# inhavl-shlee/AFI-GAN

Hardware: AMD Instinct MI355X
Metric: stage1_G+D_step_images_per_s (higher is better)
Workload: dtype f32 via f16x3: two scaled fp16 pieces per operand, three f16 MFMAs per product, fp32 accumulate (tensors fp32)

## Files before the change

### afigan_amd/csrc/nets.hip

```cpp
#include <string.h>
#include <stdlib.h>

#include "../../include/afigan_hip.h"
#include "afi_common.h"
#include "afi_launch.h"
#include <initializer_list>
#include <new>


#include <vector>
namespace {
struct SideStream {
    hipStream_t side = nullptr;
    std::vector<hipEvent_t> ring;
    size_t next = 0;
    bool init() {
        if (side) return true;
        if (hipStreamCreateWithFlags(&side, hipStreamNonBlocking) != hipSuccess) { side = nullptr; return false; }
        ring.resize(128);
        for (auto& e : ring)
            if (hipEventCreateWithFlags(&e, hipEventDisableTiming) != hipSuccess) return false;
        return true;
    }
    void destroy() {
// ... 247 lines not shown
    int nj = 0;
    long long used = 0;
    for (int i = 0; i < n; ++i) {
        const Wk6Req& r = reqs[i];
        const long long need = wk6_req_floats(r.Ncols, r.Ck, r.nKphase);
        bool hit = false;
        float* slot = wino_wcache_slot(cx, r.key,  4 + r.tag, r.nKphase, r.Ncols, r.Ck, need, hit);
        if (!slot) {
            if (!arena || used + need > arena_floats) { im.n = 0; return AFI_OK; }
            slot = arena + used; used += need; hit = false;
        }
        const int nst = afi_cdiv(r.Ck, 32) * 9 * r.nKphase;
        if (!hit && r.convT) {
            if (have_ct) { im.n = 0; return AFI_OK; }
            ct = AfiWk6ConvT{r.j[0].src, (unsigned char*)slot, r.pack_dst, r.convT == 1 ? r.Ck : r.Ncols, r.convT == 1 ? r.Ncols / 4 : r.Ck, r.convT == 1 ? 0 : 1, 0};
            have_ct = true;
        } else if (!hit) {
            int chunk0 = 0;
            for (int k = 0; k < r.njob; ++k) {
                if (nj == kWk6MaxJobs) { im.n = 0; return AFI_OK; }
                jobs[nj++] = AfiWk6ImgJob{r.j[k].src, r.j[k].b_sRow, r.j[k].b_sTap, r.Ncols, r.j[k].Ck, 9, r.nKphase, r.b_rc, chunk0 * 9 * r.nKphase,
                                          (unsigned char*)slot, r.njob > 1 ? nst : 0, 0};
                chunk0 += afi_cdiv(r.j[k].Ck, 32);
            }
        }
        im.e[im.n++] = Wk6Images::Ent{r.key, r.tag, (const unsigned char*)slot, nst};
    }
    if (nj || have_ct) {
        AFI_TRY(afi_launch_wk6_images(jobs, nj, st, side, have_ct ? &ct : nullptr));
        if (side && side_done) *side_done = true;
        if (have_ct && ct_built) *ct_built = true;
    }
    rollback.keep = true;
    im.on = true;
    return AFI_OK;
}
static inline bool wk6_shapes_ok(int C, int G, int R) { return (C % 32) == 0 && (G % 32) == 0 && 6 * R + 4 <= kWk6MaxReq && 9 * R + 4 <= kWk6MaxJobs; }
constexpr long long kWk6HiResMaxPixels = 4096;
static long long gen_wk6_fwd_floats(int C, int G, int R, long long P) {
    if (P > kWk6MaxPixels || !wk6_shapes_ok(C, G, R)) return 0;
    const int L = C + 4 * G;
    long long f = 3 * wk6_req_floats(C, C, 1) + wk6_req_floats(4 * C, C, 1);
    for (int k = 1; k <= 4; ++k) f += (long long)R * wk6_req_floats(G, C + (k - 1) * G, 1);
    return f + (long long)R * wk6_req_floats(C, L, 1);
}
static long long gen_wk6_bwd_floats(int C, int G, int R, long long P) {
    if (P > kWk6MaxPixels || !wk6_shapes_ok(C, G, R)) return 0;
    const int L = C + 4 * G;
    long long f = 3 * wk6_req_floats(C, C, 1) + wk6_req_floats(C, C, 4);
    for (int k = 1; k <= 4; ++k) f += (long long)R * wk6_req_floats(C + (k - 1) * G, G, 1);
    return f + (long long)R * (wk6_req_floats(L, C, 1) + wk6_req_floats(C, 4 * G, 1));
}

static int wino_run(afi_ctx* cx, const AfiPixGemm& g, const WinoForm& f, float* ws, long long ws_floats, float* part, long long part_floats, hipStream_t st) {
    AFI_TRY(afi_o16_refused(g));
    const int b_rc = f.kind == kWinoDgrad;
    const int nph = g.nKphase;
    const int K = g.Ck * nph, Nc = g.Ncols;
    if (ws_floats < wino_ws_floats(g.N, g.H, g.W, K, Nc)) return AFI_ERR_WORKSPACE;
    const int dtype = f.dtype, np = f.np; const long long Tpad = f.Tpad;
    const bool f4 = f.f4, dma = f.dma, f16 = f.f16;
    float* U = ws;
    float* Vb = U + align4((long long)np * K * Nc);
    float* Mb = Vb + align4(np * Tpad * K);
    float* Usp = Mb + align4(np * Tpad * Nc);
    float* amax = nullptr;
    bool have_u = false;
    if (g.no_wcache) {
    } else if (dma) {
        if (float* slot = wino_wcache_slot(cx, g.B, f4, b_rc | (dtype << 4), b_rc ? K : Nc, b_rc ? Nc : K, wino_usplit_floats(np, (long long)K * Nc), have_u)) Usp = slot;
    } else if (float* slot = wino_wcache_slot(cx, g.B, f4, b_rc, b_rc ? K : Nc, b_rc ? Nc : K, align4((long long)np * K * Nc), have_u)) U = slot;
    if (!have_u) {
        float* wmax = dma && f16 ? afi_f16_image_wmax(Usp) : nullptr;
        if (wmax) AFI_TRY(afi_f16_image_begin(Usp, st));
        AFI_TRY(f4 ? afi_launch_wino4_weight(g.B, U, b_rc ? K : Nc, b_rc ? Nc : K, b_rc, st, wmax)
                   : afi_launch_wino_weight(g.B, U, b_rc ? K : Nc, b_rc ? Nc : K, b_rc, st, wmax));
        if (dma) AFI_TRY(f16 ? afi_launch_split_f16_tiles(U, Usp, np, Nc, K, st, f4 ? 6 : 5) : afi_launch_split_bf16_tiles(U, Usp, np, Nc, K, dtype, st));
    }
    const bool a_pre = f.presplit && g.a_amax && g.a_amax_known;
    if (f16 && !(amax = g.a_amax ? g.a_amax : wino_amax_take(cx, ws, ws_floats, 1, st))) return AFI_ERR_LAUNCH;
    const AfiF16Bound abound = afi_f16_bound(amax, f4 ? 2 : 1);
    if (g.v_keep && !(f.keep && a_pre)) return AFI_ERR_BAD_ARG;
    if (g.v_keep) Vb = g.v_keep;
    for (int ph = 0; ph < nph; ++ph) {
        AfiView a = g.A;
        if (nph == 4) { a.p += (ph >> 1) * g.A.sH + (ph & 1) * g.A.sW; a.sH *= 2; a.sW *= 2; }
        float* raise = g.a_amax ? (g.a_amax_known ? nullptr : g.a_amax) : (f16 ? amax : nullptr);
        AFI_TRY(f4 ? afi_launch_wino4_input(a, g.N, g.H, g.W, g.Ck, Tpad, Vb + ph * g.Ck, st, K, &g.a_bn, raise, a_pre ? &abound : nullptr)
                   : afi_launch_wino_input(a, g.N, g.H, g.W, g.Ck, Tpad, Vb + ph * g.Ck, st, K, &g.a_bn, raise, a_pre ? &abound : nullptr));
    }
    if (dma) {
        if (f16) AFI_TRY(afi_launch_gemm_nt_f16x3(Vb, Usp, Mb, np, Tpad, Nc, K, abound, st, a_pre, afi_opt(cx, AFI_OPT_F16_NT256_MIN_TILES), g.nt_local_sums != 0));
        else AFI_TRY(afi_launch_gemm_nt_bf16_dma(Vb, Usp, Mb, np, Tpad, Nc, K, dtype, st));
        return f4 ? afi_launch_wino4_output_epi(Mb, Tpad, g, st) : afi_launch_wino_output_epi(Mb, Tpad, g, st);
    }
    if (dtype == AFI_DTYPE_F32) {
        const int rc = afi_launch_gemm_nt(Vb, U, Mb, np, Tpad, Nc, K, st);
        if (rc == AFI_OK) return f4 ? afi_launch_wino4_output_epi(Mb, Tpad, g, st) : afi_launch_wino_output_epi(Mb, Tpad, g, st);
        if (rc != AFI_ERR_UNSUPPORTED) return rc;
    }
    AfiPixGemm q = pix_default(np, 1, (int)Tpad);
    q.ntaps = 1; q.Ck = K; q.Ncols = Nc; q.CoutPhase = Nc;
    q.A = AfiView{Vb, Tpad * K, 0, K};
    q.B = U; q.b_sRow = K; q.b_sTap = 0; q.b_sImg = (long long)K * Nc;
    q.n_fastest = 1;
    q.O = AfiView{Mb, Tpad * Nc, 0, Nc};
    q.partial = part; q.partial_floats = part_floats;
    AFI_TRY(afi_launch_pix_gemm(q, 0, st));
    return f4 ? afi_launch_wino4_output_epi(Mb, Tpad, g, st) : afi_launch_wino_output_epi(Mb, Tpad, g, st);
}

struct AfiBwdSums { double* rows; const float* c; AfiBnLoad bn; float slope; };
struct WinoConvOpt {
    double* stats = nullptr; float* stats_mm = nullptr; int* stats_rows = nullptr;
    const AfiBnLoad* in_bn = nullptr;
    float* in_amax = nullptr; bool in_amax_known = false;
    float* v_keep = nullptr;
    bool local_sums = false;
    const AfiBwdSums* bsums = nullptr; int* bsums_rows = nullptr;
};
static int wino_conv(afi_ctx* cx, WinoKind kind, AfiView in, int N, int H, int W, int K, const float* w, int Nc, const float* bias, AfiView out, AfiView z,
// ... 281 lines not shown
    AFI_CTX_CHECK(ctx);
    if (out_dtype != AFI_STORE_BF16 && out_dtype != AFI_STORE_F16) return AFI_ERR_BAD_ARG;
    if ((Cin & 3) || (Cout & 3)) return AFI_ERR_UNSUPPORTED;
    AfiPixGemm g = conv_fwd_desc(V(x), N, H, W, Cin, w, bias, Cout, V(out));
    g.alpha = alpha; g.beta = beta; g.lrelu = lrelu; g.o_dtype = out_dtype;
    return launch_pix_op(cx, g, 0, (hipStream_t)stream);
}
int afi_conv3x3_dgrad(afi_ctx_t* ctx, afi_view_t dy, int N, int H, int W, int Cout, const float* w, int Cin, afi_view_t dx, float alpha, float beta,
                      afi_view_t z, void* stream) {
    afi_ctx* cx = ctx; (void)cx;
    AFI_CTX_CHECK(ctx);
    if ((Cin & 3) || (Cout & 3)) return AFI_ERR_UNSUPPORTED;
    AfiPixGemm g = conv_dgrad_desc(V(dy), N, H, W, Cout, w, Cin, V(dx));
    g.alpha = alpha; g.beta = beta;
    if (z.p) { g.Z = V(z); g.z_lo = 0; g.z_hi = Cin; }
    return launch_pix_op(cx, g, 1, (hipStream_t)stream);
}
int afi_conv3x3_wgrad(afi_ctx_t* ctx, afi_view_t dy, afi_view_t x, int N, int H, int W, int Cout, int Cin, float* dw, float alpha, void* stream) {
    afi_ctx* cx = ctx; (void)cx;
    AFI_CTX_CHECK(ctx);
    if ((Cin & 3) || (Cout & 3)) return AFI_ERR_UNSUPPORTED;
    return wgrad_launch(cx, conv_wgrad_desc(V(dy), V(x), N, H, W, Cout, Cin, dw, alpha), (hipStream_t)stream);
}

long long afi_conv3x3_wino_ws_floats(int N, int H, int W, int Cin, int Cout) { return wino_ws_floats(N, H, W, Cin, Cout); }
int afi_conv3x3_wino_fwd(afi_ctx_t* ctx, afi_view_t x, int N, int H, int W, int Cin, const float* w, const float* bias, int Cout, afi_view_t out, float* ws,
                         long long ws_floats, void* stream) {
    afi_ctx* cx = ctx; (void)cx;
    AFI_CTX_CHECK(ctx);
    if (N <= 0 || H <= 0 || W <= 0 || !ws) return AFI_ERR_BAD_ARG;
    return wino_conv(cx, kWinoFwd, V(x), N, H, W, Cin, w, Cout, bias, V(out), null_view(), ws, ws_floats, nullptr, 0, (hipStream_t)stream);
}
int afi_conv3x3_wino_fwd_out16(afi_ctx_t* ctx, afi_view_t x, int N, int H, int W, int Cin, const float* w, const float* bias, int Cout, afi_view_t out,
                               int out_dtype, float* ws, long long ws_floats, void* stream) {
    afi_ctx* cx = ctx; (void)cx;
    AFI_CTX_CHECK(ctx);
    if (out_dtype != AFI_STORE_BF16 && out_dtype != AFI_STORE_F16) return AFI_ERR_BAD_ARG;
    if (N <= 0 || H <= 0 || W <= 0 || !ws) return AFI_ERR_BAD_ARG;
    if ((Cin & 3) || (Cout & 3)) return AFI_ERR_UNSUPPORTED;
    AfiPixGemm g = conv_fwd_desc(V(x), N, H, W, Cin, w, bias, Cout, V(out));
    g.o_dtype = out_dtype;
    return wino_run(cx, g, wino_form(cx, g, 0), ws, ws_floats, nullptr, 0, (hipStream_t)stream);
}
int afi_conv3x3_wino_infer(afi_ctx_t* ctx, afi_view_t x, int N, int H, int W, int Cin, const float* w, const float* bias, int Cout, afi_view_t out, int act,
                           float* ws, long long ws_floats, void* stream) {
    afi_ctx* cx = ctx; (void)cx;
    AFI_CTX_CHECK(ctx);
    if (N <= 0 || H <= 0 || W <= 0 || !ws || act < 0 || act > 2) return AFI_ERR_BAD_ARG;
    if ((Cin & 3) || (Cout & 3)) return AFI_ERR_UNSUPPORTED;
    AfiPixGemm g = conv_fwd_desc(V(x), N, H, W, Cin, w, bias, Cout, V(out));
    g.lrelu = act;
    return wino_run(cx, g, wino_form(cx, g, 0, true), ws, ws_floats, nullptr, 0, (hipStream_t)stream);
}
int afi_conv3x3_wino_dgrad(afi_ctx_t* ctx, afi_view_t dy, int N, int H, int W, int Cout, const float* w, int Cin, afi_view_t dx, afi_view_t z, float* ws,
                           long long ws_floats, void* stream) {
    afi_ctx* cx = ctx; (void)cx;
    AFI_CTX_CHECK(ctx);
    if (N <= 0 || H <= 0 || W <= 0 || !ws) return AFI_ERR_BAD_ARG;
    return wino_conv(cx, kWinoDgrad, V(dy), N, H, W, Cout, w, Cin, nullptr, V(dx), z.p ? V(z) : null_view(), ws, ws_floats, nullptr, 0, (hipStream_t)stream);
}

int afi_conv3x3_wino_wgrad(afi_ctx_t* ctx, afi_view_t dy, afi_view_t x, int N, int H, int W, int Cout, int Cin, float* dw, float alpha, float* ws,
                           long long ws_floats, void* stream) {
    afi_ctx* cx = ctx; (void)cx;
    AFI_CTX_CHECK(ctx);
    if (N <= 0 || H <= 0 || W <= 0 || !ws || !dw) return AFI_ERR_BAD_ARG;
    return wino_wgrad(cx, V(dy), V(x), N, H, W, Cout, Cin, dw, alpha, ws, ws_floats, (hipStream_t)stream);
}

int afi_conv1x1_fwd(afi_ctx_t* ctx, afi_view_t x, int N, int H, int W, int Cin, const float* w, const float* bias, int Cout, afi_view_t out, float alpha,
                    float beta, afi_view_t r1, float r1_scale, int lrelu, void* stream) {
    afi_ctx* cx = ctx; (void)cx;
    AFI_CTX_CHECK(ctx);
    if ((Cin & 3) || (Cout & 3)) return AFI_ERR_UNSUPPORTED;
    AfiPixGemm g = pix_default(N, H, W);
    g.ntaps = 1; g.Ck = Cin; g.Ncols = Cout; g.CoutPhase = Cout;
    g.A = V(x); g.B = w; g.b_sRow = Cin; g.b_sTap = 0;
    g.O = V(out); g.bias = bias; g.alpha = alpha; g.beta = beta; g.lrelu = lrelu;
    if (r1.p) { g.R1 = V(r1); g.r1s = r1_scale; g.r1_lo = 0; g.r1_hi = Cout; }
    return launch_pix_op(cx, g, 0, (hipStream_t)stream);
}
int afi_conv1x1_dgrad(afi_ctx_t* ctx, afi_view_t dy, int N, int H, int W, int Cout, const float* w, int Cin, afi_view_t dx, float alpha, float beta,
                      void* stream) {
    afi_ctx* cx = ctx; (void)cx;
    AFI_CTX_CHECK(ctx);
    if ((Cin & 3) || (Cout & 3)) return AFI_ERR_UNSUPPORTED;
    AfiPixGemm g = pix_default(N, H, W);
    g.ntaps = 1; g.a_sgn = -1; g.Ck = Cout; g.Ncols = Cin; g.CoutPhase = Cin;
    g.A = V(dy); g.B = w; g.b_sRow = Cin; g.b_sTap = 0;
    g.O = V(dx); g.alpha = alpha; g.beta = beta;
    return launch_pix_op(cx, g, 1, (hipStream_t)stream);
}
int afi_conv1x1_dgrad_out16(afi_ctx_t* ctx, afi_view_t dy, int N, int H, int W, int Cout, const float* w, int Cin, afi_view_t dx, int dx_dtype, float alpha,
                            float beta, void* stream) {
    afi_ctx* cx = ctx; (void)cx;
    AFI_CTX_CHECK(ctx);
    if (dx_dtype != AFI_STORE_BF16 && dx_dtype != AFI_STORE_F16) return AFI_ERR_BAD_ARG;
    if ((Cin & 3) || (Cout & 3)) return AFI_ERR_UNSUPPORTED;
    AfiPixGemm g = pix_default(N, H, W);
    g.ntaps = 1; g.a_sgn = -1; g.Ck = Cout; g.Ncols = Cin; g.CoutPhase = Cin;
    g.A = V(dy); g.B = w; g.b_sRow = Cin; g.b_sTap = 0;
    g.O = V(dx); g.alpha = alpha; g.beta = beta; g.o_dtype = dx_dtype;
    return launch_pix_op(cx, g, 1, (hipStream_t)stream);
}
int afi_conv1x1_wgrad(afi_ctx_t* ctx, afi_view_t dy, afi_view_t x, int N, int H, int W, int Cout, int Cin, float* dw, float alpha, void* stream) {
    afi_ctx* cx = ctx; (void)cx;
// ... 1133 lines not shown
```

### afigan_amd/guide.py

```python
import math

import torch
import torch.nn as nn
import torch.nn.functional as F

from . import ops


def _kaiming(shape, fan_in, gain=1.0):
    return torch.randn(shape) * (gain * math.sqrt(2.0 / fan_in))


class _Conv1x1(nn.Module):
    def __init__(self, cin, cout, stride=1, relu=False, gain=1.0):
        super().__init__()
        self.stride, self.relu = stride, relu
        self.register_buffer("w", _kaiming((cin, cout), cin, gain).t().contiguous())
        self.register_buffer("b", torch.zeros(cout))

    def forward(self, x, add=None, relu=None):
        if self.stride != 1:
            x = x[:, :, ::self.stride, ::self.stride]
        return ops.conv1x1_fwd(x, self.w, self.b, add=add, act=2 if (self.relu if relu is None else relu) else 0)


class _Conv3x3(nn.Module):
    def __init__(self, cin, cout, relu=False):
        super().__init__()
        self.relu = relu
        self.register_buffer("w", _kaiming((cout, 3, 3, cin), cin * 9).permute(0, 3, 1, 2))
        self.register_buffer("b", torch.zeros(cout))

    def forward(self, x):
        N, C, H, W = x.shape
        if C >= 128 and self.w.shape[0] >= 128 and N * H * W >= 1024:
            return ops.conv3x3_wino_infer(x, self.w, self.b, act=2 if self.relu else 0)
        return ops.conv3x3_fwd(x, self.w, self.b, lrelu=2 if self.relu else 0)


class _Bottleneck(nn.Module):
    def __init__(self, cin, mid, cout, stride):
        super().__init__()
        self.c1 = _Conv1x1(cin, mid, stride, relu=True)
        self.c2 = _Conv3x3(mid, mid, relu=True)
        self.c3 = _Conv1x1(mid, cout, gain=0.25)
        self.short = _Conv1x1(cin, cout, stride) if (cin != cout or stride != 1) else None

    def forward(self, x):
        s = x if self.short is None else self.short(x)
        return self.c3(self.c2(self.c1(x)), add=s, relu=True)


class GuideR50FPN(nn.Module):

    def __init__(self, out_channels=256):
        super().__init__()
        self.register_buffer("stem_w", _kaiming((3 * 49, 64), 3 * 49))
        self.register_buffer("stem_b", torch.zeros(64))
        cfg = [(64, 64, 256, 3, 1), (256, 128, 512, 4, 2), (512, 256, 1024, 6, 2), (1024, 512, 2048, 3, 2)]
        self.stages = nn.ModuleList()
        for cin, mid, cout, n, stride in cfg:
            blocks = [_Bottleneck(cin, mid, cout, stride)] + [_Bottleneck(cout, mid, cout, 1) for _ in range(n - 1)]
            self.stages.append(nn.Sequential(*blocks))
        self.lateral = nn.ModuleList([_Conv1x1(c, out_channels, gain=0.1) for c in (256, 512, 1024, 2048)])
        self.output = nn.ModuleList([_Conv3x3(out_channels, out_channels) for _ in range(4)])
        self.register_buffer("pixel_mean", torch.tensor([103.53, 116.28, 123.675]).view(1, 3, 1, 1))
        self.eval()

    @torch.no_grad()
    def forward(self, images):
        x = (images - self.pixel_mean) * (1.0 / 58.0)
        H, W = x.shape[-2:]
        ph, pw = (32 - H % 32) % 32, (32 - W % 32) % 32
        if ph or pw:
            x = F.pad(x, (0, pw, 0, ph))
        N, _, H, W = x.shape
        cols = F.unfold(x, kernel_size=7, padding=3, stride=2)
        y = F.relu_(torch.baddbmm(self.stem_b.view(1, 1, -1), cols.transpose(1, 2), self.stem_w.unsqueeze(0).expand(N, -1, -1)))
        x = y.view(N, H // 2, W // 2, 64).permute(0, 3, 1, 2)
        x = F.max_pool2d(x, 3, 2, 1).contiguous(memory_format=torch.channels_last)
        feats = []
        for st in self.stages:
            x = st(x)
            feats.append(x)
        prev = self.lateral[3](feats[3])
        outs = [self.output[3](prev)]
        for i in (2, 1, 0):
            up = F.interpolate(prev, scale_factor=2, mode="nearest")
            prev = self.lateral[i](feats[i], add=up)
            outs.insert(0, self.output[i](prev))
        outs.append(outs[-1][:, :, ::2, ::2].contiguous(memory_format=torch.channels_last))
        return {f"p{i + 2}": o for i, o in enumerate(outs)}
```

### afigan_amd/ops.py

```python
import contextlib
import ctypes as C
import os

import torch

from . import _lib
from ._lib import View, call

_NULL_VIEW = View(None, 0, 0, 0)


def stream_ptr():
    return C.c_void_p(torch.cuda.current_stream().cuda_stream)


def _check_cuda(*ts):
    for t in ts:
        if t is None:
            continue
        if not t.is_cuda:
            raise _lib.AfiError("the AFI-GAN hot path runs on the GPU only (got a CPU tensor); there is no CPU fallback")
        if t.dtype != torch.float32:
            raise _lib.AfiError(f"fp32 only on this path, got {t.dtype}")

# ... 225 lines not shown
    return out


def conv3x3_dgrad(dy, w, dx=None, alpha=1.0, beta=0.0, z=None):
    _check_cuda(dy, w, dx, z)
    _ensure_op_scratch(dy.device)
    N, Cout, H, W = dy.shape
    Cin = w.shape[1]
    w = ohwi(w)
    if dx is None:
        dx = new_pixel_major(N, Cin, H, W, dy.device)
    call("afi_conv3x3_dgrad", view_of(dy), N, H, W, Cout, _p(w), Cin, view_of(dx), float(alpha), float(beta),
         view_of(z) if z is not None else _NULL_VIEW, stream_ptr())
    return dx


def conv3x3_wgrad(dy, x, dw=None, alpha=1.0):
    _check_cuda(dy, x, dw)
    N, Cout, H, W = dy.shape
    Cin = x.shape[1]
    if dw is None:
        dw = new_ohwi(Cout, Cin, 3, 3, dy.device)
    assert dw.permute(0, 2, 3, 1).is_contiguous()
    call("afi_conv3x3_wgrad", view_of(dy), view_of(x), N, H, W, Cout, Cin, _p(dw), float(alpha), stream_ptr())
    return dw


def conv3x3_wino_fwd(x, w, bias=None, out_dtype=torch.float32):
    _check_cuda(x, w, bias)
    N, Cin, H, W = x.shape
    Cout = w.shape[0]
    w = ohwi(w)
    n = _lib.load().afi_conv3x3_wino_ws_floats(N, H, W, Cin, Cout)
    ws = new_workspace(n, x.device)
    out = new_pixel_major(N, Cout, H, W, x.device, dtype=out_dtype)
    if out_dtype != torch.float32:
        call("afi_conv3x3_wino_fwd_out16", view_of(x), N, H, W, Cin, _p(w), _p(bias), Cout, view_of(out), STORE_DTYPES[out_dtype], _p(ws), n,
             stream_ptr())
        return out
    call("afi_conv3x3_wino_fwd", view_of(x), N, H, W, Cin, _p(w), _p(bias), Cout, view_of(out), _p(ws), n, stream_ptr())
    return out


def conv3x3_wino_infer(x, w, bias=None, act=0):
    _check_cuda(x, w, bias)
    N, Cin, H, W = x.shape
    Cout = w.shape[0]
    w = ohwi(w)
    n = _lib.load().afi_conv3x3_wino_ws_floats(N, H, W, Cin, Cout)
    ws = new_workspace(n, x.device)
    out = new_pixel_major(N, Cout, H, W, x.device)
    call("afi_conv3x3_wino_infer", view_of(x), N, H, W, Cin, _p(w), _p(bias), Cout, view_of(out), int(act), _p(ws), n, stream_ptr())
    return out


def conv3x3_wino_dgrad(dy, w, z=None):
    _check_cuda(dy, w, z)
    N, Cout, H, W = dy.shape
    Cin = w.shape[1]
    w = ohwi(w)
    n = _lib.load().afi_conv3x3_wino_ws_floats(N, H, W, Cin, Cout)
    ws = new_workspace(n, dy.device)
    dx = new_pixel_major(N, Cin, H, W, dy.device)
    call("afi_conv3x3_wino_dgrad", view_of(dy), N, H, W, Cout, _p(w), Cin, view_of(dx), view_of(z) if z is not None else _NULL_VIEW,
         _p(ws), n, stream_ptr())
    return dx


def conv3x3_wino_wgrad(dy, x, dw=None, alpha=1.0):
    _check_cuda(dy, x, dw)
    N, Cout, H, W = dy.shape
    Cin = x.shape[1]
    if dw is None:
        dw = new_ohwi(Cout, Cin, 3, 3, dy.device)
    assert dw.permute(0, 2, 3, 1).is_contiguous()
    n = _lib.load().afi_conv3x3_wino_ws_floats(N, H, W, Cin, Cout)
    ws = new_workspace(n, dy.device)
    call("afi_conv3x3_wino_wgrad", view_of(dy), view_of(x), N, H, W, Cout, Cin, _p(dw), float(alpha), _p(ws), n, stream_ptr())
    return dw


def conv3x3s2_fwd(x, w, bias=None, act=0, add=None, add_scale=1.0, post_scale=1.0, keep_act=False):
    _check_cuda(x, w, bias, add)
    _ensure_op_scratch(x.device)
    N, Cin, Hi, Wi = x.shape
    Cout = w.shape[0]
    w = ohwi(w)
    Ho, Wo = (Hi + 1) // 2, (Wi + 1) // 2
    if add is not None and tuple(add.shape) != (N, Cout, Ho, Wo):
        raise _lib.AfiError(f"conv3x3s2_fwd: residual shape {tuple(add.shape)} != {(N, Cout, Ho, Wo)}")
    out = new_pixel_major(N, Cout, Ho, Wo, x.device)
    a = new_pixel_major(N, Cout, Ho, Wo, x.device) if keep_act else None
    call("afi_conv3x3s2_fwd", view_of(x), N, Hi, Wi, Cin, _p(w), _p(bias), Cout, view_of(out), int(act),
         view_of(a) if a is not None else _NULL_VIEW, float(post_scale), view_of(add) if add is not None else _NULL_VIEW,
         float(add_scale), stream_ptr())
    return (out, a) if keep_act else out


def conv3x3s2_dgrad(dy, w, in_hw, dx=None, alpha=1.0, beta=0.0):
    _check_cuda(dy, w, dx)
    _ensure_op_scratch(dy.device)
    N, Cout, Ho, Wo = dy.shape
    Hi, Wi = in_hw
    if ((Hi + 1) // 2, (Wi + 1) // 2) != (Ho, Wo):
        raise _lib.AfiError(f"conv3x3s2_dgrad: dy {Ho}x{Wo} is not the stride-2 output of {Hi}x{Wi}")
    Cin = w.shape[1]
# ... 669 lines not shown
```

### include/afigan_hip.h

```cpp
#ifndef AFIGAN_HIP_H
#define AFIGAN_HIP_H

#include <stddef.h>
#include <stdint.h>

#ifdef __cplusplus
extern "C" {
#endif

#define AFI_OK 0
#define AFI_ERR_BAD_ARG 1
#define AFI_ERR_UNSUPPORTED 2
#define AFI_ERR_LAUNCH 3
#define AFI_ERR_WORKSPACE 4

#define AFI_MAX_RDB 8

typedef struct afi_view {
    float* p;
    long long sN, sH, sW;
} afi_view_t;

int afi_abi_version(void);
const char* afi_status_string(int status);
// ... 73 lines not shown

typedef struct afi_disc_params {
    int F[4];
    float* w[3]; float* b[3];
    float* gamma[3]; float* beta[3];
    float* running_mean[3]; float* running_var[3];
    long long* num_batches_tracked[3];
    float* w3; float* b3;
} afi_disc_params_t;

long long afi_discriminator_fwd_ws_floats(const int F[4], int N, int H, int W);
long long afi_discriminator_fwd_ws_floats_ex(const afi_ctx_t* ctx, const int F[4], int N, int H, int W, int training);
long long afi_discriminator_bwd_ws_floats(const int F[4], int N, int H, int W);
int afi_discriminator_ws_layout(const int F[4], int N, int H, int W, long long* off12);
int afi_discriminator_saved_activations(const afi_ctx_t* ctx, const int F[4], int N, int H, int W);

int afi_discriminator_fwd(afi_ctx_t* ctx, const afi_disc_params_t* prm, afi_view_t x, int N, int H, int W, float* logits, int training,
                          float* ws, long long ws_floats, void* stream);
int afi_discriminator_bwd(afi_ctx_t* ctx, const afi_disc_params_t* prm, const afi_disc_params_t* grads, afi_view_t x, int N, int H, int W,
                          const float* ws, const float* dlogits, float* dx, float* scratch, long long scratch_floats, void* stream);

int afi_discriminator_fwd_paired(afi_ctx_t* ctx, const afi_disc_params_t* prm, afi_view_t x, int N, int H, int W, float* logits, int training,
                                 float* ws, long long ws_floats, void* stream);
int afi_discriminator_bwd_paired(afi_ctx_t* ctx, const afi_disc_params_t* prm, const afi_disc_params_t* grads, afi_view_t x, int N, int H, int W,
                                 const float* ws, const float* dlogits, float* dx, float* scratch, long long scratch_floats, void* stream);


int afi_conv3x3_fwd(afi_ctx_t* ctx, afi_view_t x, int N, int H, int W, int Cin, const float* w, const float* bias, int Cout,
                    afi_view_t out, float alpha, float beta, int lrelu, void* stream);
int afi_conv3x3_dgrad(afi_ctx_t* ctx, afi_view_t dy, int N, int H, int W, int Cout, const float* w, int Cin, afi_view_t dx,
                      float alpha, float beta, afi_view_t z_or_null, void* stream);
int afi_conv3x3_wgrad(afi_ctx_t* ctx, afi_view_t dy, afi_view_t x, int N, int H, int W, int Cout, int Cin, float* dw, float alpha, void* stream);
int afi_conv3x3_fwd_out16(afi_ctx_t* ctx, afi_view_t x, int N, int H, int W, int Cin, const float* w, const float* bias, int Cout,
                          afi_view_t out, int out_dtype, float alpha, float beta, int lrelu, void* stream);

int afi_conv1x1_fwd(afi_ctx_t* ctx, afi_view_t x, int N, int H, int W, int Cin, const float* w, const float* bias, int Cout, afi_view_t out,
                    float alpha, float beta, afi_view_t r1_or_null, float r1_scale, int lrelu, void* stream);
int afi_conv1x1_dgrad(afi_ctx_t* ctx, afi_view_t dy, int N, int H, int W, int Cout, const float* w, int Cin, afi_view_t dx, float alpha, float beta,
                      void* stream);
int afi_conv1x1_wgrad(afi_ctx_t* ctx, afi_view_t dy, afi_view_t x, int N, int H, int W, int Cout, int Cin, float* dw, float alpha, void* stream);
int afi_conv1x1_dgrad_out16(afi_ctx_t* ctx, afi_view_t dy, int N, int H, int W, int Cout, const float* w, int Cin, afi_view_t dx, int dx_dtype,
                            float alpha, float beta, void* stream);

long long afi_conv3x3_wino_ws_floats(int N, int H, int W, int Cin, int Cout);
int afi_conv3x3_wino_fwd(afi_ctx_t* ctx, afi_view_t x, int N, int H, int W, int Cin, const float* w_ohwi, const float* bias_or_null, int Cout,
                         afi_view_t out, float* ws, long long ws_floats, void* stream);
int afi_conv3x3_wino_fwd_out16(afi_ctx_t* ctx, afi_view_t x, int N, int H, int W, int Cin, const float* w_ohwi, const float* bias_or_null, int Cout,
                               afi_view_t out, int out_dtype, float* ws, long long ws_floats, void* stream);
int afi_conv3x3_wino_infer(afi_ctx_t* ctx, afi_view_t x, int N, int H, int W, int Cin, const float* w_ohwi, const float* bias_or_null, int Cout,
                           afi_view_t out, int act, float* ws, long long ws_floats, void* stream);
int afi_conv3x3_wino_dgrad(afi_ctx_t* ctx, afi_view_t dy, int N, int H, int W, int Cout, const float* w_ohwi, int Cin, afi_view_t dx,
                           afi_view_t z_or_null, float* ws, long long ws_floats, void* stream);

int afi_conv3x3_wino_wgrad(afi_ctx_t* ctx, afi_view_t dy, afi_view_t x, int N, int H, int W, int Cout, int Cin, float* dw, float alpha, float* ws,
                           long long ws_floats, void* stream);

int afi_conv3x3s2_fwd(afi_ctx_t* ctx, afi_view_t x, int N, int Hi, int Wi, int Cin, const float* w_ohwi, const float* bias_or_null, int Cout,
                      afi_view_t out, int act, afi_view_t act_out_or_null, float post_scale, afi_view_t r_or_null, float r_scale,
                      void* stream);
int afi_conv3x3s2_dgrad(afi_ctx_t* ctx, afi_view_t dy , int N, int Hi, int Wi, int Cout, const float* w_ohwi, int Cin,
                        afi_view_t dx, float alpha, float beta, void* stream);
int afi_conv3x3s2_wgrad(afi_ctx_t* ctx, afi_view_t dy, afi_view_t x , int N, int Hi, int Wi, int Cout, int Cin, float* dw,
                        float alpha, void* stream);
int afi_relu_bwd(const float* g, const float* act, float* out, long long n, float scale, void* stream);

int afi_dwconv3x3_fwd(afi_view_t x, int N, int H, int W, int C, const float* w9c, float* out, void* stream);
int afi_maxpool3s2_same_fwd(afi_view_t x, int N, int H, int W, int C, float* out, void* stream);
int afi_fuse_swish_fwd(const float* a, const float* b, const float* c_or_null, const float* w_dev, float* out, long long n,
                       void* stream);

long long afi_fuse_swish_bwd_scratch_floats(void);
int afi_fuse_swish_bwd(const float* a, const float* b, const float* c_or_null, const float* w_dev, const float* dout, float* da_or_null,
                       float* db_or_null, float* dc_or_null, float* dw_or_null, long long n, float* scratch, void* stream);
long long afi_dwconv3x3_wgrad_scratch_floats(int C);
int afi_dwconv3x3_wgrad(const float* dy, const float* x, int N, int H, int W, int C, float* dw9c, float* scratch, void* stream);
int afi_maxpool3s2_same_fwd_idx(afi_view_t x, int N, int H, int W, int C, float* out, unsigned char* idx, void* stream);
int afi_maxpool3s2_same_bwd(const float* dout, const unsigned char* idx, int N, int H, int W, int C, float* dx, void* stream);

int afi_convT6s2_pack_weight(const float* w_iohw, float* wp, int Cin, int Cout, void* stream);
int afi_convT6s2_unpack_wgrad(const float* dwp, float* dw_iohw, int Cin, int Cout, void* stream);
int afi_convT6s2_fwd(afi_ctx_t* ctx, afi_view_t x, int N, int H, int W, int Cin, const float* wp, const float* bias, int Cout,
                     afi_view_t out , int lrelu, void* stream);
int afi_convT6s2_dgrad(afi_ctx_t* ctx, afi_view_t dy , int N, int H, int W, int Cout, const float* wp, int Cin,
                       afi_view_t dx, afi_view_t z_or_null, void* stream);
int afi_convT6s2_wgrad(afi_ctx_t* ctx, afi_view_t dy, afi_view_t x, int N, int H, int W, int Cout, int Cin, float* dwp, float alpha, void* stream);

int afi_bilinear2x_add_fwd(afi_view_t x, int N, int H, int W, int C, float beta, float* out, void* stream);
int afi_bilinear2x_add_bwd(const float* dout, int N, int H, int W, int C, float beta, float* dx, void* stream);

long long afi_reduce_scratch_floats(int C);
int afi_bn_stats(const float* x, long long P, int C, float* mean, float* invstd, float* var_biased_or_null,
                 float* running_mean_or_null, float* running_var_or_null, float* scratch, void* stream);
int afi_bn_apply_lrelu_fwd(const float* x, float* y, const float* mean, const float* invstd, const float* gamma,
                           const float* beta, long long P, int C, void* stream);
int afi_bn_stats_ex(const float* x, long long P, int C, float eps, float momentum, float* mean, float* invstd, float* var_biased_or_null,
                    float* running_mean_or_null, float* running_var_or_null, long long* num_batches_tracked_or_null, float* scratch,
                    void* stream);
int afi_bn_apply_fwd(const float* x, float* y, const float* mean, const float* invstd, const float* gamma, const float* beta,
                     long long P, int C, float slope, void* stream);
int afi_bn_bwd(const float* g, const float* x, float* dx, const float* mean, const float* invstd, const float* gamma,
               float* dgamma, float* dbeta, long long P, int C, float* scratch, void* stream);
int afi_bn_bwd_sums(const float* g, const float* x, const float* mean, const float* invstd, float* dgamma_or_null, float* dbeta_or_null, float* sums2C,
                    long long P, int C, float* scratch, void* stream);
int afi_bn_bwd_apply(const float* g, const float* x, float* dx, const float* mean, const float* invstd, const float* gamma, const float* sums2C,
                     long long P, long long P_total, int C, void* stream);
int afi_colsum_accum(const float* g, long long P, int C, long long ld, float alpha, float* db, float* scratch, void* stream);
// ... 85 lines not shown
```

Measured before the change: 28.61.

## Add frozen 3x3 conv handle with prebuilt f16 Winograd weight images for guide net

Adds a persistent frozen-conv handle that builds the Winograd-transformed, f16-split weight images for the frozen guide network once, and reuses them on every forward. Each call also draws a per-call amax slot from a device ring. The guide module now uses these handles and shares one workspace across calls, keyed by input shape, instead of allocating per call. This removes per-call weight transform and split launches and workspace allocation. The cost is extra device memory and staleness logic that must be refreshed when the weights change.

Measured after the change: 28.43. No clear change (-0.6%).

```diff
diff --git a/afigan_amd/csrc/nets.hip b/afigan_amd/csrc/nets.hip
--- a/afigan_amd/csrc/nets.hip
+++ b/afigan_amd/csrc/nets.hip
@@ -323,7 +323,8 @@
     return f + (long long)R * (wk6_req_floats(L, C, 1) + wk6_req_floats(C, 4 * G, 1));
 }
 
-static int wino_run(afi_ctx* cx, const AfiPixGemm& g, const WinoForm& f, float* ws, long long ws_floats, float* part, long long part_floats, hipStream_t st) {
+static int wino_run(afi_ctx* cx, const AfiPixGemm& g, const WinoForm& f, float* ws, long long ws_floats, float* part, long long part_floats, hipStream_t st,
+                    float* u_img = nullptr) {
     AFI_TRY(afi_o16_refused(g));
     const int b_rc = f.kind == kWinoDgrad;
     const int nph = g.nKphase;
@@ -337,7 +338,8 @@
     float* Usp = Mb + align4(np * Tpad * Nc);
     float* amax = nullptr;
     bool have_u = false;
-    if (g.no_wcache) {
+    if (u_img) { Usp = u_img; have_u = true; }
+    else if (g.no_wcache) {
     } else if (dma) {
         if (float* slot = wino_wcache_slot(cx, g.B, f4, b_rc | (dtype << 4), b_rc ? K : Nc, b_rc ? Nc : K, wino_usplit_floats(np, (long long)K * Nc), have_u)) Usp = slot;
     } else if (float* slot = wino_wcache_slot(cx, g.B, f4, b_rc, b_rc ? K : Nc, b_rc ? Nc : K, align4((long long)np * K * Nc), have_u)) U = slot;
@@ -725,6 +727,130 @@
     g.lrelu = act;
     return wino_run(cx, g, wino_form(cx, g, 0, true), ws, ws_floats, nullptr, 0, (hipStream_t)stream);
 }
+namespace {
+constexpr unsigned kFrozenAlive = 0xaf1f07e9u, kFrozenDead = 0xdeadf07eu;
+inline long long align256(long long n) { return (n + 255) & ~255LL; }
+}
+struct afi_frozen_conv {
+    unsigned magic;
+    int kind, Cin, Cout, device, dtype;
+    const float* w; const float* bias;
+    unsigned char* base; long long bytes;
+    long long off_img[2], img_bytes[2], off_u;
+    long long off_ring; int ring_next;
+};
+constexpr int kFrozenSlots = 64;
+constexpr long long kFrozenRingBytes = 16LL * kFrozenSlots;
+static inline bool frozen_live(const afi_frozen_conv* h) { return h && h->magic == kFrozenAlive; }
+int afi_frozen_conv_check_span(const void* base, long long base_bytes, const void* ws, long long ws_bytes, const void* p, long long bytes) {
+    if (!p || bytes <= 0) return AFI_ERR_BAD_ARG;
+    const unsigned long long a = (unsigned long long)(size_t)p, n = (unsigned long long)bytes;
+    if (a + n < a) return AFI_ERR_BAD_ARG;
+    auto inside = [&](const void* b, long long nb) {
+        if (!b || nb <= 0) return false;
+        const unsigned long long lo = (unsigned long long)(size_t)b, hi = lo + (unsigned long long)nb;
+        return hi >= lo && a >= lo && a + n <= hi;
+    };
+    return inside(base, base_bytes) || inside(ws, ws_bytes) ? AFI_OK : AFI_ERR_BAD_ARG;
+}
+static int frozen_build(afi_frozen_conv* h, hipStream_t st) {
+    if (!h->base) return AFI_OK;
+    float* U = (float*)(h->base + h->off_u);
+    if (afi_frozen_conv_check_span(h->base, h->bytes, nullptr, 0, h->base + h->off_ring, kFrozenRingBytes) != AFI_OK) return AFI_ERR_BAD_ARG;
+    if (hipMemsetAsync(h->base + h->off_ring, 0, kFrozenRingBytes, st) != hipSuccess) return AFI_ERR_LAUNCH;
+    h->ring_next = 0;
+    for (int f4 = 1; f4 >= 0; --f4) {
+        unsigned char* img = h->base + h->off_img[f4];
+        const int np = f4 ? 36 : 16;
+        if (afi_frozen_conv_check_span(h->base, h->bytes, nullptr, 0, img, h->img_bytes[f4]) != AFI_OK ||
+            afi_frozen_conv_check_span(h->base, h->bytes, nullptr, 0, U, 4LL * np * h->Cin * h->Cout) != AFI_OK) return AFI_ERR_BAD_ARG;
+        AFI_TRY(afi_f16_image_begin(img, st));
+        AFI_TRY(f4 ? afi_launch_wino4_weight(h->w, U, h->Cout, h->Cin, 0, st, afi_f16_image_wmax(img))
+                   : afi_launch_wino_weight(h->w, U, h->Cout, h->Cin, 0, st, afi_f16_image_wmax(img)));
+        AFI_TRY(afi_launch_split_f16_tiles(U, img, np, h->Cout, h->Cin, st, f4 ? 6 : 5));
+    }
+    return AFI_OK;
+}
+int afi_frozen_conv_create(afi_ctx_t* ctx, int kind, const float* w, const float* bias, int Cin, int Cout, void* stream, afi_frozen_conv_t** handle) {
+    if (!handle) return AFI_ERR_BAD_ARG;
+    *handle = nullptr;
+    if (!w || Cin <= 0 || Cout <= 0 || (kind != AFI_FROZEN_CONV1X1 && kind != AFI_FROZEN_CONV3X3)) return AFI_ERR_BAD_ARG;
+    if (kind == AFI_FROZEN_CONV1X1 || (Cin & 3) || (Cout & 3)) return AFI_ERR_UNSUPPORTED;
+    AFI_CTX_CHECK(ctx);
+    afi_frozen_conv* h = new (std::nothrow) afi_frozen_conv();
+    if (!h) return AFI_ERR_WORKSPACE;
+    h->kind = kind; h->Cin = Cin; h->Cout = Cout; h->w = w; h->bias = bias;
+    h->dtype = ctx ? ctx->dtype : afi_default_dtype();
+    h->base = nullptr; h->bytes = 0;
+    if (hipGetDevice(&h->device) != hipSuccess) { delete h; return AFI_ERR_LAUNCH; }
+    if (h->dtype == AFI_DTYPE_F16X3 && Cin >= 128 && Cout >= 128 && !(Cout % 128) && !(Cin % 32)) {
+        h->img_bytes[1] = afi_f16_image_bytes(36, Cout, Cin); h->img_bytes[0] = afi_f16_image_bytes(16, Cout, Cin);
+        h->off_img[1] = 0; h->off_img[0] = align256(h->img_bytes[1]);
+        h->off_u = h->off_img[0] + align256(h->img_bytes[0]);
+        h->off_ring = h->off_u + align256(4LL * 36 * Cin * Cout);
+        h->bytes = h->off_ring + kFrozenRingBytes;
+        void* p = nullptr;
+        if (hipMalloc(&p, (size_t)h->bytes) != hipSuccess || !p) { (void)hipGetLastError(); delete h; return AFI_ERR_WORKSPACE; }
+        h->base = (unsigned char*)p;
+    }
+    h->magic = kFrozenAlive;
+    const int rc = frozen_build(h, (hipStream_t)stream);
+    if (rc != AFI_OK) { (void)afi_frozen_conv_destroy(h); delete h; return rc; }
+    *handle = h;
+    return AFI_OK;
+}
+int afi_frozen_conv_refresh(afi_frozen_conv_t* h, const float* w, const float* bias, void* stream) {
+    if (!frozen_live(h) || !w) return AFI_ERR_BAD_ARG;
+    int d = -1;
+    if (hipGetDevice(&d) != hipSuccess || d != h->device) return AFI_ERR_BAD_ARG;
+    h->w = w; h->bias = bias;
+    return frozen_build(h, (hipStream_t)stream);
+}
+int afi_frozen_conv_destroy(afi_frozen_conv_t* h) {
+    if (!frozen_live(h)) return AFI_ERR_BAD_ARG;
+    h->magic = kFrozenDead;
+    if (h->base) (void)hipFree(h->base);
+    h->base = nullptr; h->bytes = 0; h->w = h->bias = nullptr;
+    return AFI_OK;
+}
+long long afi_frozen_conv_device_bytes(const afi_frozen_conv_t* h) { return frozen_live(h) ? h->bytes : -1; }
+int afi_frozen_conv3x3_fwd(afi_ctx_t* ctx, afi_frozen_conv_t* h, afi_view_t x, int N, int H, int W, afi_view_t out, int act, float* ws, long long ws_floats,
+                           void* stream) {
+    if (!frozen_live(h) || h->kind != AFI_FROZEN_CONV3X3) return AFI_ERR_BAD_ARG;
+    if (!x.p || !out.p || N <= 0 || H <= 0 || W <= 0 || act < 0 || act > 2 || ws_floats < 0) return AFI_ERR_BAD_ARG;
+    afi_ctx* cx = ctx;
+    AFI_CTX_CHECK(ctx);
+    int d = -1;
+    if (hipGetDevice(&d) != hipSuccess || d != h->device) return AFI_ERR_BAD_ARG;
+    hipStream_t st = (hipStream_t)stream;
+    const int K = h->Cin, Nc = h->Cout;
+    AfiPixGemm g = conv_fwd_desc(V(x), N, H, W, K, h->w, h->bias, Nc, V(out));
+    g.lrelu = act;
+    if (K < 128 || Nc < 128 || (long long)N * H * W < 1024) return launch_pix_op(cx, g, 0, st);
+    if (!ws) return AFI_ERR_BAD_ARG;
+    const WinoForm f = wino_form(cx, g, 0, true);
+    if (!h->base || !f.dma || !f.f16 || f.dtype != h->dtype) return wino_run(cx, g, f, ws, ws_floats, nullptr, 0, st);
+    if (ws_floats < wino_ws_floats(N, H, W, K, Nc)) return AFI_ERR_WORKSPACE;
+    unsigned char* img = h->base + h->off_img[f.f4 ? 1 : 0];
+    const long long wsb = 4 * ws_floats;
+    float* Vb = ws + align4((long long)f.np * K * Nc);
+    float* Mb = Vb + align4(f.np * f.Tpad * K);
+    float* ring = (float*)(h->base + h->off_ring);
+    if (h->ring_next >= kFrozenSlots) {
+        if (hipMemsetAsync(ring, 0, kFrozenRingBytes, st) != hipSuccess) return AFI_ERR_LAUNCH;
+        h->ring_next = 0;
+    }
+    float* slot = ring + 4 * h->ring_next;
+    if (afi_frozen_conv_check_span(h->base, h->bytes, nullptr, 0, img, afi_f16_image_bytes(f.np, Nc, K)) != AFI_OK ||
+        afi_frozen_conv_check_span(h->base, h->bytes, nullptr, 0, afi_f16_image_wmax(img), 4) != AFI_OK ||
+        afi_frozen_conv_check_span(nullptr, 0, ws, wsb, Vb, 4 * f.np * f.Tpad * K) != AFI_OK ||
+        afi_frozen_conv_check_span(nullptr, 0, ws, wsb, Mb, 4 * f.np * f.Tpad * Nc) != AFI_OK ||
+        afi_frozen_conv_check_span(h->base, h->bytes, nullptr, 0, slot, 16) != AFI_OK) return AFI_ERR_BAD_ARG;
+    h->ring_next++;
+    g.a_amax = slot; g.a_amax_known = 0;
+    return wino_run(cx, g, f, ws, ws_floats, nullptr, 0, st, (float*)img);
+}
+
 int afi_conv3x3_wino_dgrad(afi_ctx_t* ctx, afi_view_t dy, int N, int H, int W, int Cout, const float* w, int Cin, afi_view_t dx, afi_view_t z, float* ws,
                            long long ws_floats, void* stream) {
     afi_ctx* cx = ctx; (void)cx;
diff --git a/afigan_amd/guide.py b/afigan_amd/guide.py
--- a/afigan_amd/guide.py
+++ b/afigan_amd/guide.py
@@ -25,17 +25,50 @@
 
 
 class _Conv3x3(nn.Module):
+
     def __init__(self, cin, cout, relu=False):
         super().__init__()
         self.relu = relu
         self.register_buffer("w", _kaiming((cout, 3, 3, cin), cin * 9).permute(0, 3, 1, 2))
         self.register_buffer("b", torch.zeros(cout))
+        self._frozen, self._stale = None, False
+        self._wsbox = [None]
+
+    def refresh(self):
+        self._stale = True
+
+    def __getstate__(self):
+        d = dict(self.__dict__)
+        d["_frozen"], d["_stale"] = None, False
+        return d
+
+    def _drop(self):
+        if self._frozen is not None:
+            self._frozen.destroy()
+            self._frozen = None
+        self._stale = False
+
+    def _load_from_state_dict(self, *args, **kw):
+        super()._load_from_state_dict(*args, **kw)
+        self._stale = True
+
+    def _apply(self, fn, *args, **kw):
+        self._drop()
+        return super()._apply(fn, *args, **kw)
+
+    def __del__(self):
+        try:
+            self._drop()
+        except Exception:
+            pass
 
     def forward(self, x):
-        N, C, H, W = x.shape
-        if C >= 128 and self.w.shape[0] >= 128 and N * H * W >= 1024:
-            return ops.conv3x3_wino_infer(x, self.w, self.b, act=2 if self.relu else 0)
-        return ops.conv3x3_fwd(x, self.w, self.b, lrelu=2 if self.relu else 0)
+        if self._frozen is None:
+            self._frozen = ops.FrozenConv3x3(self.w, self.b)
+        elif self._stale:
+            self._frozen.refresh(self.w, self.b)
+        self._stale = False
+        return self._frozen.forward(x, act=2 if self.relu else 0, ws=self._wsbox[0])
 
 
 class _Bottleneck(nn.Module):
@@ -65,7 +98,25 @@
         self.lateral = nn.ModuleList([_Conv1x1(c, out_channels, gain=0.1) for c in (256, 512, 1024, 2048)])
         self.output = nn.ModuleList([_Conv3x3(out_channels, out_channels) for _ in range(4)])
         self.register_buffer("pixel_mean", torch.tensor([103.53, 116.28, 123.675]).view(1, 3, 1, 1))
+        self._wsbox = [None]
+        self._ws = {}
+        for m in self.modules():
+            if isinstance(m, _Conv3x3):
+                m._wsbox = self._wsbox
         self.eval()
+
+    def _workspace(self, N, H, W, device):
+        key = (N, H, W, str(device))
+        ws = self._ws.get(key)
+        if ws is None:
+            lib, n = ops._lib.load(), 64
+            for lvl, st in enumerate(self.stages):
+                h, w = H >> (2 + lvl), W >> (2 + lvl)
+                mid = st[0].c2.w.shape[0]
+                cout = self.output[lvl].w.shape[0]
+                n = max(n, lib.afi_conv3x3_wino_ws_floats(N, h, w, mid, mid), lib.afi_conv3x3_wino_ws_floats(N, h, w, cout, cout))
+            ws = self._ws[key] = ops.new_workspace(n, device)
+        return ws
 
     @torch.no_grad()
     def forward(self, images):
@@ -75,6 +126,7 @@
         if ph or pw:
             x = F.pad(x, (0, pw, 0, ph))
         N, _, H, W = x.shape
+        self._wsbox[0] = self._workspace(N, H, W, x.device)
         cols = F.unfold(x, kernel_size=7, padding=3, stride=2)
         y = F.relu_(torch.baddbmm(self.stem_b.view(1, 1, -1), cols.transpose(1, 2), self.stem_w.unsqueeze(0).expand(N, -1, -1)))
         x = y.view(N, H // 2, W // 2, 64).permute(0, 3, 1, 2)
diff --git a/afigan_amd/ops.py b/afigan_amd/ops.py
--- a/afigan_amd/ops.py
+++ b/afigan_amd/ops.py
@@ -301,6 +301,61 @@
     out = new_pixel_major(N, Cout, H, W, x.device)
     call("afi_conv3x3_wino_infer", view_of(x), N, H, W, Cin, _p(w), _p(bias), Cout, view_of(out), int(act), _p(ws), n, stream_ptr())
     return out
+
+
+class FrozenConv3x3:
+
+    def __init__(self, w, bias=None):
+        _check_cuda(w, bias)
+        if not w.permute(0, 2, 3, 1).is_contiguous():
+            raise _lib.AfiError("FrozenConv3x3: the weight must already live as [O][3][3][I] (the handle reads it in place)")
+        self.w, self.bias = w, bias
+        self.handle = C.c_void_p()
+        with torch.cuda.device(w.device):
+            _lib.check(_lib.load().afi_frozen_conv_create(_lib.current_ctx().handle, _lib.DEFINES["AFI_FROZEN_CONV3X3"], _p(w), _p(bias), w.shape[1],
+                                                          w.shape[0], stream_ptr(), C.byref(self.handle)), "afi_frozen_conv_create")
+
+    def refresh(self, w=None, bias=None):
+        w = self.w if w is None else w
+        bias = self.bias if bias is None else bias
+        _check_cuda(w, bias)
+        if w.shape != self.w.shape or w.device != self.w.device or not w.permute(0, 2, 3, 1).is_contiguous():
+            raise _lib.AfiError("FrozenConv3x3.refresh: same shape, device and [O][3][3][I] memory only (make a new handle otherwise)")
+        with torch.cuda.device(w.device):
+            call("afi_frozen_conv_refresh", self.handle, _p(w), _p(bias), stream_ptr())
+        self.w, self.bias = w, bias
+
+    def ws_floats(self, N, H, W):
+        return int(_lib.load().afi_conv3x3_wino_ws_floats(N, H, W, self.w.shape[1], self.w.shape[0]))
+
+    def forward(self, x, act=0, ws=None):
+        _check_cuda(x, ws)
+        _ensure_op_scratch(x.device)
+        N, Cin, H, W = x.shape
+        if not self.handle or Cin != self.w.shape[1] or x.device != self.w.device:
+            raise _lib.AfiError(f"FrozenConv3x3: input {tuple(x.shape)} on {x.device} does not fit this handle (destroyed, other channels or device)")
+        if Cin >= 128 and self.w.shape[0] >= 128 and N * H * W >= 1024:
+            n = self.ws_floats(N, H, W)
+            if ws is None or ws.numel() < n:
+                ws = new_workspace(n, x.device)
+        else:
+            ws = None
+        out = new_pixel_major(N, self.w.shape[0], H, W, x.device)
+        call("afi_frozen_conv3x3_fwd", _lib.current_ctx().handle, self.handle, view_of(x), N, H, W, view_of(out), int(act), _p(ws),
+             ws.numel() if ws is not None else 0, stream_ptr())
+        return out
+
+    def destroy(self):
+        if self.handle:
+            call("afi_frozen_conv_destroy", self.handle)
+            self.handle = C.c_void_p()
+            self.w = self.bias = None
+
+    def __del__(self):
+        try:
+            self.destroy()
+        except Exception:
+            pass
 
 
 def conv3x3_wino_dgrad(dy, w, z=None):
diff --git a/include/afigan_hip.h b/include/afigan_hip.h
--- a/include/afigan_hip.h
+++ b/include/afigan_hip.h
@@ -149,6 +149,18 @@
 int afi_conv3x3_wino_dgrad(afi_ctx_t* ctx, afi_view_t dy, int N, int H, int W, int Cout, const float* w_ohwi, int Cin, afi_view_t dx,
                            afi_view_t z_or_null, float* ws, long long ws_floats, void* stream);
 
+typedef struct afi_frozen_conv afi_frozen_conv_t;
+#define AFI_FROZEN_CONV1X1 1
+#define AFI_FROZEN_CONV3X3 3
+int afi_frozen_conv_create(afi_ctx_t* ctx, int kind, const float* w, const float* bias_or_null, int Cin, int Cout, void* stream,
+                           afi_frozen_conv_t** handle);
+int afi_frozen_conv_refresh(afi_frozen_conv_t* handle, const float* w, const float* bias_or_null, void* stream);
+int afi_frozen_conv_destroy(afi_frozen_conv_t* handle);
+long long afi_frozen_conv_device_bytes(const afi_frozen_conv_t* handle);
+int afi_frozen_conv3x3_fwd(afi_ctx_t* ctx, afi_frozen_conv_t* handle, afi_view_t x, int N, int H, int W, afi_view_t out, int act, float* ws,
+                           long long ws_floats, void* stream);
+int afi_frozen_conv_check_span(const void* base, long long base_bytes, const void* ws, long long ws_bytes, const void* p, long long bytes);
+
 int afi_conv3x3_wino_wgrad(afi_ctx_t* ctx, afi_view_t dy, afi_view_t x, int N, int H, int W, int Cout, int Cin, float* dw, float alpha, float* ws,
                            long long ws_floats, void* stream);
 
```
